# Dhia-naouali/dinov3-jax

Hardware: NVIDIA H100
Metric: global_crops_per_sec (higher is better)
Workload: dtype bf16

## Files before the change

### dinov3-jax_b200/csrc/attention.cu

```cuda
#include "ptx.cuh"
#include <climits>
#include <cstdlib>
#include "d3_internal.h"

namespace d3 {

constexpr float LOG2E = 1.4426950408889634f;
constexpr int SMEM_ALIGN = 1024;

__device__ __forceinline__ uint8_t* smem_base_1024(uint8_t* raw) {
  return reinterpret_cast<uint8_t*>((reinterpret_cast<uintptr_t>(raw) + 1023) & ~uintptr_t(1023));
}

struct AttnShape {
  int G;
  int span;
  int n_crops;
  int N;
  int nkb;
  int D;
  int H;
  float scale;
  const float* sin_t;
  const float* cos_t;
// ... 2 lines not shown

__device__ __forceinline__ uint32_t sw128_offset(int row, int col) {
  return (uint32_t)(row * 128 + ((((col >> 3) ^ (row & 7)) & 7) << 4) + (col & 7) * 2);
}

struct RowInfo { int g, klo, khi; bool ok; };
__device__ __forceinline__ RowInfo row_info(const AttnShape& sh, int c, int q) {
  RowInfo ri;
  ri.g = min(q / sh.N, sh.G - 1);
  ri.klo = ri.g * sh.N;
  ri.khi = ri.klo + sh.N;
  ri.ok = (q < sh.span) && (c * sh.G + ri.g < sh.n_crops);
  return ri;
}

template <int NI, int NO>
__device__ __forceinline__ void online_softmax(float (&s)[4 * NI], float (&o)[NO], float (&m)[2], float (&l)[2],
                                               const RowInfo (&ri)[2], int k0, int c2, float cs) {
  const int kb0 = k0 + c2;
  const bool full = k0 >= max(ri[0].klo, ri[1].klo) && k0 + 8 * NI <= min(ri[0].khi, ri[1].khi);
  float mx[2] = {-3.0e38f, -3.0e38f};
#pragma unroll
  for (int i = 0; i < NI; ++i)
#pragma unroll
    for (int j = 0; j < 4; ++j) {
      const int hh = j >> 1, kk = kb0 + 8 * i + (j & 1);
      if (full || (kk >= ri[hh].klo && kk < ri[hh].khi)) mx[hh] = fmaxf(mx[hh], s[4 * i + j]);
    }
  float corr[2], ms[2];
#pragma unroll
  for (int hh = 0; hh < 2; ++hh) {
    mx[hh] = fmaxf(mx[hh], __shfl_xor_sync(0xffffffffu, mx[hh], 1));
    mx[hh] = fmaxf(mx[hh], __shfl_xor_sync(0xffffffffu, mx[hh], 2));
    const float mn = fmaxf(m[hh], mx[hh]);
    corr[hh] = ex2_approx((m[hh] - mn) * cs);
    m[hh] = mn;
    ms[hh] = mn * cs;
    l[hh] *= corr[hh];
  }
#pragma unroll
  for (int i = 0; i < NI; ++i)
#pragma unroll
    for (int j = 0; j < 4; ++j) {
      const int hh = j >> 1, kk = kb0 + 8 * i + (j & 1);
      const float p = (full || (kk >= ri[hh].klo && kk < ri[hh].khi)) ? ex2_approx(fmaf(s[4 * i + j], cs, -ms[hh])) : 0.f;
      s[4 * i + j] = p;
      l[hh] += p;
      if (i < NO / 4) o[4 * i + j] *= corr[hh];
    }
}

template <int NO>
__device__ __forceinline__ void store_o_lse(const float (&o)[NO], float (&l)[2], const float (&m)[2], const RowInfo (&ri)[2],
                                            const AttnShape& sh, int c, int h, int row_base, int wq0, int r_in, int c2,
                                            __nv_bfloat16* O, float* LSE) {
#pragma unroll
  for (int hh = 0; hh < 2; ++hh) {
    l[hh] += __shfl_xor_sync(0xffffffffu, l[hh], 1);
    l[hh] += __shfl_xor_sync(0xffffffffu, l[hh], 2);
    const int q = wq0 + r_in + 8 * hh;
    if (!ri[hh].ok) continue;
    const float inv = 1.f / l[hh];
    __nv_bfloat16* dst = O + (size_t)(row_base + q) * sh.D + h * (2 * NO) + c2;
#pragma unroll
    for (int i = 0; i < NO / 4; ++i)
      *reinterpret_cast<uint32_t*>(dst + 8 * i) = pack_bf16(o[4 * i + 2 * hh] * inv, o[4 * i + 2 * hh + 1] * inv);
    if (LSE && c2 == 0)
      LSE[((size_t)(c * sh.G + ri[hh].g) * sh.H + h) * sh.N + (q - ri[hh].klo)] = m[hh] * sh.scale + logf(l[hh]);
  }
}

__host__ __device__ constexpr int fwd_smem(int nkb) { return SMEM_ALIGN + 16384 + 2 * nkb * 8192 + 8; }

__global__ void __launch_bounds__(256)
attn_fwd_kernel(const __grid_constant__ CUtensorMap tmQ, const __grid_constant__ CUtensorMap tmKV,
                __nv_bfloat16* __restrict__ O, float* __restrict__ LSE, const AttnShape sh) {
  extern __shared__ uint8_t smem_raw[];
  uint8_t* sQ = smem_base_1024(smem_raw);
  uint8_t* sK = sQ + 16384;
  uint8_t* sV = sK + sh.nkb * 8192;
  uint64_t* bar = reinterpret_cast<uint64_t*>(sV + sh.nkb * 8192);

  const int wg = threadIdx.x >> 7, t = threadIdx.x & 127;
  const int qt = blockIdx.x, h = blockIdx.y, c = blockIdx.z;
  const int q0 = qt * 128;
  const int row_base = c * sh.span;
  if (threadIdx.x == 0) {
    tma_prefetch_desc(&tmQ);
    tma_prefetch_desc(&tmKV);
    mbar_init(bar, 1);
    fence_mbar_init();
  }
  __syncthreads();
  if (threadIdx.x < 32 && elect_one()) {
    mbar_expect_tx(bar, 16384 + 2 * sh.nkb * 8192);
    tma_load_2d(&tmQ, bar, sQ, h * 64, row_base + q0);
    for (int b = 0; b < sh.nkb; ++b) {
      tma_load_2d(&tmKV, bar, sK + b * 8192, sh.D + h * 64, row_base + b * 64);
      tma_load_2d(&tmKV, bar, sV + b * 8192, 2 * sh.D + h * 64, row_base + b * 64);
    }
  }
  const int wq0 = q0 + wg * 64;
  if (wq0 >= sh.span) return;
  mbar_wait(bar, 0);

  const int r_in = 16 * (t >> 5) + ((t & 31) >> 2), c2 = 2 * (t & 3);
  RowInfo ri[2];
  ri[0] = row_info(sh, c, wq0 + r_in);
  ri[1] = row_info(sh, c, wq0 + r_in + 8);
  const int b_lo = (min(wq0 / sh.N, sh.G - 1) * sh.N) >> 6;
  const int b_hi = min(sh.nkb, ((min(min(wq0 + 63, sh.span - 1) / sh.N, sh.G - 1) + 1) * sh.N + 63) >> 6);
  const float cs = sh.scale * LOG2E;
  float m[2] = {-3.0e38f, -3.0e38f}, l[2] = {0.f, 0.f};
  float o[32];
#pragma unroll
  for (int i = 0; i < 32; ++i) o[i] = 0.f;
  const uint64_t qd = gmma_desc_sw128(smem_u32(sQ + wg * 8192), 16, 1024);

#pragma unroll 1
  for (int b = b_lo; b < b_hi; ++b) {
    float s[32];
    const uint64_t kd = gmma_desc_sw128(smem_u32(sK + b * 8192), 16, 1024);
    fence_regs(o);
    wgmma_fence();
#pragma unroll
    for (int k = 0; k < 4; ++k) wgmma_m64n64k16_ss<0, 0>(s, qd + 2 * k, kd + 2 * k, k > 0 ? 1u : 0u);
    wgmma_commit();
    wgmma_wait<0>();
    fence_regs(s);
    online_softmax<8>(s, o, m, l, ri, b * 64, c2, cs);
    uint32_t a[4][4];
#pragma unroll
    for (int kk = 0; kk < 4; ++kk)
#pragma unroll
      for (int e = 0; e < 4; ++e) a[kk][e] = pack_bf16(s[8 * kk + 2 * e], s[8 * kk + 2 * e + 1]);
    const uint64_t vd = gmma_desc_sw128(smem_u32(sV + b * 8192), 8192, 1024);
    fence_regs(o);
    wgmma_fence();
#pragma unroll
    for (int kk = 0; kk < 4; ++kk) wgmma_m64n64k16_rs<1>(o, a[kk], vd + 128 * kk, 1u);
    wgmma_commit();
    wgmma_wait<0>();
    fence_regs(o);
  }
  store_o_lse(o, l, m, ri, sh, c, h, row_base, wq0, r_in, c2, O, LSE);
}

template <int STAGES, int BYTES>
struct TileRing {
  static constexpr int SMEM = STAGES * BYTES + 2 * STAGES * 8;
  uint8_t* buf;
  uint64_t* full;
  uint64_t* empty;

  __device__ __forceinline__ explicit TileRing(uint8_t* base)
// ... 258 lines not shown
#pragma unroll
  for (int kk = 0; kk < 8; ++kk)
#pragma unroll
    for (int e = 0; e < 4; ++e) a[kk][e] = pack_bf16(dp[8 * kk + 2 * e], dp[8 * kk + 2 * e + 1]);
  const uint64_t kd = gmma_desc_sw128(smem_u32(sK), 8192, 1024);
  fence_regs(dq);
  wgmma_fence();
#pragma unroll
  for (int kk = 0; kk < 8; ++kk) wgmma_m64n64k16_rs<1>(dq, a[kk], kd + 128 * kk, 1u);
  wgmma_commit();
  wgmma_wait<0>();
  fence_regs(dq);
}


__host__ __device__ constexpr int bwd_fused_smem(int n_t) {
  return n_t * 32768 * 2 + 32768 + (n_t > 1 ? 2 * 32768 : 0) + n_t * 128 * 8 + 2 * n_t * 8;
}

__device__ __forceinline__ uint64_t desc_here(const void* p, uint32_t lbo, uint32_t sbo) {
  uint32_t a;
  asm volatile("mov.b32 %0, %1;" : "=r"(a) : "r"(smem_u32(p)));
  return gmma_desc_sw128(a, lbo, sbo);
}

template <int R>
__device__ __forceinline__ void fence_frag(uint32_t (&a)[R][4]) {
#pragma unroll
  for (int i = 0; i < R; ++i)
#pragma unroll
    for (int e = 0; e < 4; ++e) asm volatile("" : "+r"(a[i][e])::"memory");
}

__global__ void __launch_bounds__(256, 1)
attn_bwd_fused_kernel(const __grid_constant__ CUtensorMap tmQKV, const __grid_constant__ CUtensorMap tmDO,
                      const float* __restrict__ LSE, const float* __restrict__ Delta, __nv_bfloat16* __restrict__ dQKV,
                      const AttnShape sh) {
  extern __shared__ __align__(1024) uint8_t smem_al[];
  const int nT = (sh.span + 127) / 128;
  uint8_t* sKV = smem_al;
  uint8_t* sQDO = sKV + nT * 32768;
  uint8_t* sDS = sQDO + nT * 32768;
  uint8_t* sDS0 = sDS + 32768;
  float* sDQ = reinterpret_cast<float*>(sDS0 + 32768);
  float* sLSE = reinterpret_cast<float*>(sDS + (nT > 1 ? 3 * 32768 : 32768));
  float* sDel = sLSE + nT * 128;
  uint64_t* bar_kv = reinterpret_cast<uint64_t*>(sDel + nT * 128);
  uint64_t* bar_q = bar_kv + nT;

  const int wg = threadIdx.x >> 7, t = threadIdx.x & 127;
  const int r_in = 16 * (t >> 5) + ((t & 31) >> 2), c2 = 2 * (t & 3);
  const int h = blockIdx.x, c = blockIdx.y;
  const int row_base = c * sh.span;
  if (threadIdx.x == 0) {
    tma_prefetch_desc(&tmQKV);
    tma_prefetch_desc(&tmDO);
    for (int i = 0; i < 2 * nT; ++i) mbar_init(bar_kv + i, 1);
    fence_mbar_init();
  }
  __syncthreads();
  if (threadIdx.x < 32 && elect_one()) {
    for (int i = 0; i < nT; ++i) {
      mbar_expect_tx(bar_kv + i, 32768);
      tma_load_2d(&tmQKV, bar_kv + i, sKV + i * 32768, sh.D + h * 64, row_base + i * 128);
      tma_load_2d(&tmQKV, bar_kv + i, sKV + i * 32768 + 16384, 2 * sh.D + h * 64, row_base + i * 128);
      mbar_expect_tx(bar_q + i, 32768);
      tma_load_2d(&tmQKV, bar_q + i, sQDO + i * 32768, h * 64, row_base + i * 128);
      tma_load_2d(&tmDO, bar_q + i, sQDO + i * 32768 + 16384, h * 64, row_base + i * 128);
    }
  }
  for (int q = threadIdx.x; q < nT * 128; q += 256) {
    const RowInfo ri = row_info(sh, c, q);
    const size_t stat = ((size_t)(c * sh.G + ri.g) * sh.H + h) * sh.N + (q - ri.klo);
    sLSE[q] = ri.ok ? LSE[stat] * LOG2E : 0.f;
    sDel[q] = ri.ok ? Delta[stat] : 0.f;
  }
  __syncthreads();

  const float cs = sh.scale * LOG2E;
  int pair = 0;
#pragma unroll 1
  for (int kt = 0; kt < nT; ++kt) {
    mbar_wait(bar_kv + kt, 0);
    const uint8_t* sK = sKV + kt * 32768;
    const uint8_t* sV = sK + 16384;
    int lo[2], hi[2];
#pragma unroll
    for (int hh = 0; hh < 2; ++hh) {
      const RowInfo ri = row_info(sh, c, kt * 128 + wg * 64 + r_in + 8 * hh);
      lo[hh] = ri.ok ? ri.klo : 0;
      hi[hh] = ri.ok ? ri.khi : 0;
    }
    float dk[32], dv[32];
#pragma unroll 1
    for (int qt = 0; qt < nT; ++qt, ++pair) {
      mbar_wait(bar_q + qt, 0);
      const uint8_t* sQt = sQDO + qt * 32768;
      const uint8_t* sDOt = sQt + 16384;
      const bool defer = nT == 2 && kt == 0 && qt == 0;
      uint8_t* stash = defer ? sDS0 : sDS;
      uint32_t pa[2][4][4], da[2][4][4];
#pragma unroll
      for (int hf = 0; hf < 2; ++hf) {
        float s[32], dp[32];
        {
          const uint64_t kd = desc_here(sK + wg * 8192, 16, 1024);
          const uint64_t vd = desc_here(sV + wg * 8192, 16, 1024);
          const uint64_t qd = desc_here(sQt + hf * 8192, 16, 1024);
          const uint64_t dod = desc_here(sDOt + hf * 8192, 16, 1024);
          wgmma_fence();
#pragma unroll
          for (int k = 0; k < 4; ++k) {
            wgmma_m64n64k16_ss<0, 0>(s, kd + 2 * k, qd + 2 * k, k > 0 ? 1u : 0u);
            wgmma_m64n64k16_ss<0, 0>(dp, vd + 2 * k, dod + 2 * k, k > 0 ? 1u : 0u);
          }
          wgmma_commit();
          wgmma_wait<0>();
          fence_regs(s);
          fence_regs(dp);
          if (hf == 1) { fence_frag(pa[0]); fence_frag(da[0]); }
        }
        const float* lse2 = sLSE + qt * 128 + hf * 64;
        const float* del = sDel + qt * 128 + hf * 64;
#pragma unroll
        for (int i = 0; i < 8; ++i) {
          const int col = 8 * i + c2;
          const float2 l2 = *reinterpret_cast<const float2*>(lse2 + col);
          const float2 dl = *reinterpret_cast<const float2*>(del + col);
          const int q = qt * 128 + hf * 64 + col;
          float pv[4], dv4[4];
#pragma unroll
          for (int j = 0; j < 4; ++j) {
            const int hh = j >> 1, qq = q + (j & 1);
            const bool ok = qq >= lo[hh] && qq < hi[hh];
            const float p = ok ? ex2_approx(fmaf(s[4 * i + j], cs, -((j & 1) ? l2.y : l2.x))) : 0.f;
            dv4[j] = ok ? (p * sh.scale) * (dp[4 * i + j] - ((j & 1) ? dl.y : dl.x)) : 0.f;
            pv[j] = p;
          }
          pa[hf][i >> 1][2 * (i & 1)] = pack_bf16(pv[0], pv[1]);
          pa[hf][i >> 1][2 * (i & 1) + 1] = pack_bf16(pv[2], pv[3]);
          da[hf][i >> 1][2 * (i & 1)] = pack_bf16(dv4[0], dv4[1]);
          da[hf][i >> 1][2 * (i & 1) + 1] = pack_bf16(dv4[2], dv4[3]);
        }
        if (hf == 0 && pair > 1) named_bar_sync(1, 256);
#pragma unroll
        for (int hh = 0; hh < 2; ++hh)
#pragma unroll
          for (int i = 0; i < 8; ++i) {
            const uint32_t off = hf * 16384 + sw128_offset(wg * 64 + r_in + 8 * hh, 8 * i + c2);
            *reinterpret_cast<uint32_t*>(stash + off) = da[hf][i >> 1][2 * (i & 1) + hh];
          }
        {
          const uint64_t dod = desc_here(sDOt, 8192, 1024);
          const uint64_t qd = desc_here(sQt, 8192, 1024);
          const uint32_t acc_on = (qt > 0 || hf > 0) ? 1u : 0u;
          if (acc_on) { fence_regs(dk); fence_regs(dv); }
          wgmma_fence();
#pragma unroll
          for (int kk = 0; kk < 4; ++kk) {
            const int ks = 4 * hf + kk;
            wgmma_m64n64k16_rs<1>(dv, pa[hf][kk], dod + 128 * ks, (acc_on || kk > 0) ? 1u : 0u);
            wgmma_m64n64k16_rs<1>(dk, da[hf][kk], qd + 128 * ks, (acc_on || kk > 0) ? 1u : 0u);
          }
          wgmma_commit();
        }
      }
      fence_proxy_async_smem();
      if (defer) {
        wgmma_wait<0>();
        fence_regs(dk);
        fence_regs(dv);
        fence_frag(pa[1]);
        fence_frag(da[1]);
        continue;
      }
      named_bar_sync(2, 256);
      const bool from_partial = nT == 2 && kt == 1 && qt == 1;
      float dq[32];
      float4* part = reinterpret_cast<float4*>(sDQ) + wg * 8 * 128 + t;
      if (from_partial) {
#pragma unroll
        for (int j = 0; j < 8; ++j) {
          const float4 v = part[j * 128];
          dq[4 * j] = v.x; dq[4 * j + 1] = v.y; dq[4 * j + 2] = v.z; dq[4 * j + 3] = v.w;
        }
      }
      {
        const uint64_t sd = desc_here(sDS + wg * 16384, 16384, 1024);
        const uint64_t kbd = desc_here(sK, 8192, 1024);
        fence_regs(dq);
        wgmma_fence();
#pragma unroll
        for (int kk = 0; kk < 8; ++kk)
          wgmma_m64n64k16_ss<1, 1>(dq, sd + 128 * kk, kbd + 128 * kk, (from_partial || kk > 0) ? 1u : 0u);
        if (nT == 2 && kt == 1 && qt == 0) {
          const uint64_t sd0 = desc_here(sDS0 + wg * 16384, 16384, 1024);
          const uint64_t k0d = desc_here(sKV, 8192, 1024);
#pragma unroll
          for (int kk = 0; kk < 8; ++kk) wgmma_m64n64k16_ss<1, 1>(dq, sd0 + 128 * kk, k0d + 128 * kk, 1u);
        }
        wgmma_commit();
        wgmma_wait<0>();
        fence_regs(dq);
        fence_regs(dk);
        fence_regs(dv);
        fence_frag(pa[1]);
        fence_frag(da[1]);
      }
      if (nT == 2 && kt == 0) {
#pragma unroll
        for (int j = 0; j < 8; ++j) part[j * 128] = make_float4(dq[4 * j], dq[4 * j + 1], dq[4 * j + 2], dq[4 * j + 3]);
      } else {
        store_grad_rows(dq, sh, c, row_base, qt * 128 + wg * 64, r_in, c2, h, 0, true, dQKV);
      }
    }
    store_grad_rows(dk, sh, c, row_base, kt * 128 + wg * 64, r_in, c2, h, 1, true, dQKV);
    store_grad_rows(dv, sh, c, row_base, kt * 128 + wg * 64, r_in, c2, h, 2, false, dQKV);
  }
}

using DkdvRing = TileRing<DKDV_STAGES, 32768>;
constexpr int DKDV_SMEM = SMEM_ALIGN + 2 * 16384 + 2 * 32768 + DkdvRing::SMEM + 8;
using DqRing = TileRing<DQ_STAGES, 32768>;
constexpr int DQ_SMEM = SMEM_ALIGN + 2 * 16384 + DqRing::SMEM + 8;

__global__ void __launch_bounds__(RING_THREADS, 1)
attn_bwd_dkdv_kernel(const __grid_constant__ CUtensorMap tmQKV, const __grid_constant__ CUtensorMap tmDO,
                     const float* __restrict__ LSE, const float* __restrict__ Delta, __nv_bfloat16* __restrict__ dQKV,
                     const AttnShape sh) {
  extern __shared__ uint8_t smem_raw[];
  uint8_t* sK = smem_base_1024(smem_raw);
  uint8_t* sV = sK + 16384;
// ... 483 lines not shown
  if ((rc = make_map(&tdo, d_o, T, D, D, 128))) return rc;
  __nv_bfloat16* dq = (__nv_bfloat16*)dqkv;
  if (hd128) {
    if ((rc = launch<attn_bwd_dkdv_hd128_kernel>(grid, RING_THREADS, HD128_BWD_SMEM, HD128_BWD_SMEM, st, tqkv, tdo, lse,
                                                 delta_scratch, dq, s)))
      return rc;
    return launch<attn_bwd_dq_hd128_kernel>(grid, RING_THREADS, HD128_BWD_SMEM, HD128_BWD_SMEM, st, tqkv, tdo, lse,
                                            delta_scratch, dq, s);
  }
  if (streamed) {
    if ((rc = launch<attn_bwd_dkdv_kernel>(grid, RING_THREADS, DKDV_SMEM, DKDV_SMEM, st, tqkv, tdo, lse, delta_scratch, dq,
                                           s)))
      return rc;
    return launch<attn_bwd_dq_kernel>(grid, RING_THREADS, DQ_SMEM, DQ_SMEM, st, tqkv, tdo, lse, delta_scratch, dq, s);
  }
  return launch<attn_bwd_fused_kernel>(dim3(H, (n_crops + s.G - 1) / s.G), 256, bwd_fused_smem((s.span + 127) / 128),
                                       bwd_fused_smem(ATTN_BWD_RESIDENT_SPAN / 128), st, tqkv, tdo, lse, delta_scratch,
                                       dq, s);
}

}
```

### dinov3-jax_b200/csrc/ptx.cuh

```cuda
#pragma once
#include <cuda.h>
#include <cuda_runtime.h>
#include <cuda_bf16.h>
#include <stdint.h>

namespace d3 {

__device__ __forceinline__ uint32_t smem_u32(const void* p) {
  return static_cast<uint32_t>(__cvta_generic_to_shared(p));
}
__device__ __forceinline__ uint32_t lane_id() { return threadIdx.x & 31; }
__device__ __forceinline__ bool elect_one() {
  uint32_t pred;
  asm volatile("{\n\t.reg .pred p;\n\telect.sync _|p, 0xffffffff;\n\tselp.u32 %0, 1, 0, p;\n\t}" : "=r"(pred));
  return pred != 0;
}

__device__ __forceinline__ void mbar_init(uint64_t* bar, uint32_t count) {
  asm volatile("mbarrier.init.shared::cta.b64 [%0], %1;" ::"r"(smem_u32(bar)), "r"(count) : "memory");
}
__device__ __forceinline__ void fence_mbar_init() {
  asm volatile("fence.mbarrier_init.release.cluster;" ::: "memory");
}
__device__ __forceinline__ void mbar_expect_tx(uint64_t* bar, uint32_t bytes) {
// ... 107 lines not shown
__device__ __forceinline__ void wgmma_m64n32k16_ss(float (&d)[16], uint64_t da, uint64_t db, uint32_t scale_d) {
  asm volatile(
      "{\n\t.reg .pred p;\n\tsetp.ne.b32 p, %18, 0;\n\t"
      "wgmma.mma_async.sync.aligned.m64n32k16.f32.bf16.bf16 {%0, %1, %2, %3, %4, %5, %6, %7, %8, %9, %10, %11, %12, %13, %14, %15}, %16, %17, p, 1, 1, %19, %20;\n\t}"
      : "+f"(d[0]), "+f"(d[1]), "+f"(d[2]), "+f"(d[3]), "+f"(d[4]), "+f"(d[5]), "+f"(d[6]), "+f"(d[7]), "+f"(d[8]), "+f"(d[9]), "+f"(d[10]), "+f"(d[11]), "+f"(d[12]), "+f"(d[13]), "+f"(d[14]), "+f"(d[15])
      : "l"(da), "l"(db), "r"(scale_d), "n"(TA), "n"(TB));
}
template <int TA, int TB>
__device__ __forceinline__ void wgmma_m64n64k16_ss(float (&d)[32], uint64_t da, uint64_t db, uint32_t scale_d) {
  asm volatile(
      "{\n\t.reg .pred p;\n\tsetp.ne.b32 p, %34, 0;\n\t"
      "wgmma.mma_async.sync.aligned.m64n64k16.f32.bf16.bf16 {%0, %1, %2, %3, %4, %5, %6, %7, %8, %9, %10, %11, %12, %13, %14, %15, %16, %17, %18, %19, %20, %21, %22, %23, %24, %25, %26, %27, %28, %29, %30, %31}, %32, %33, p, 1, 1, %35, %36;\n\t}"
      : "+f"(d[0]), "+f"(d[1]), "+f"(d[2]), "+f"(d[3]), "+f"(d[4]), "+f"(d[5]), "+f"(d[6]), "+f"(d[7]), "+f"(d[8]), "+f"(d[9]), "+f"(d[10]), "+f"(d[11]), "+f"(d[12]), "+f"(d[13]), "+f"(d[14]), "+f"(d[15]), "+f"(d[16]), "+f"(d[17]), "+f"(d[18]), "+f"(d[19]), "+f"(d[20]), "+f"(d[21]), "+f"(d[22]), "+f"(d[23]), "+f"(d[24]), "+f"(d[25]), "+f"(d[26]), "+f"(d[27]), "+f"(d[28]), "+f"(d[29]), "+f"(d[30]), "+f"(d[31])
      : "l"(da), "l"(db), "r"(scale_d), "n"(TA), "n"(TB));
}
template <int TA, int TB>
__device__ __forceinline__ void wgmma_m64n128k16_ss(float (&d)[64], uint64_t da, uint64_t db, uint32_t scale_d) {
  asm volatile(
      "{\n\t.reg .pred p;\n\tsetp.ne.b32 p, %66, 0;\n\t"
      "wgmma.mma_async.sync.aligned.m64n128k16.f32.bf16.bf16 {%0, %1, %2, %3, %4, %5, %6, %7, %8, %9, %10, %11, %12, %13, %14, %15, %16, %17, %18, %19, %20, %21, %22, %23, %24, %25, %26, %27, %28, %29, %30, %31, %32, %33, %34, %35, %36, %37, %38, %39, %40, %41, %42, %43, %44, %45, %46, %47, %48, %49, %50, %51, %52, %53, %54, %55, %56, %57, %58, %59, %60, %61, %62, %63}, %64, %65, p, 1, 1, %67, %68;\n\t}"
      : "+f"(d[0]), "+f"(d[1]), "+f"(d[2]), "+f"(d[3]), "+f"(d[4]), "+f"(d[5]), "+f"(d[6]), "+f"(d[7]), "+f"(d[8]), "+f"(d[9]), "+f"(d[10]), "+f"(d[11]), "+f"(d[12]), "+f"(d[13]), "+f"(d[14]), "+f"(d[15]), "+f"(d[16]), "+f"(d[17]), "+f"(d[18]), "+f"(d[19]), "+f"(d[20]), "+f"(d[21]), "+f"(d[22]), "+f"(d[23]), "+f"(d[24]), "+f"(d[25]), "+f"(d[26]), "+f"(d[27]), "+f"(d[28]), "+f"(d[29]), "+f"(d[30]), "+f"(d[31]), "+f"(d[32]), "+f"(d[33]), "+f"(d[34]), "+f"(d[35]), "+f"(d[36]), "+f"(d[37]), "+f"(d[38]), "+f"(d[39]), "+f"(d[40]), "+f"(d[41]), "+f"(d[42]), "+f"(d[43]), "+f"(d[44]), "+f"(d[45]), "+f"(d[46]), "+f"(d[47]), "+f"(d[48]), "+f"(d[49]), "+f"(d[50]), "+f"(d[51]), "+f"(d[52]), "+f"(d[53]), "+f"(d[54]), "+f"(d[55]), "+f"(d[56]), "+f"(d[57]), "+f"(d[58]), "+f"(d[59]), "+f"(d[60]), "+f"(d[61]), "+f"(d[62]), "+f"(d[63])
      : "l"(da), "l"(db), "r"(scale_d), "n"(TA), "n"(TB));
}
template <int TA, int TB>
__device__ __forceinline__ void wgmma_m64n256k16_ss(float (&d)[128], uint64_t da, uint64_t db, uint32_t scale_d) {
  asm volatile(
      "{\n\t.reg .pred p;\n\tsetp.ne.b32 p, %130, 0;\n\t"
      "wgmma.mma_async.sync.aligned.m64n256k16.f32.bf16.bf16 {%0, %1, %2, %3, %4, %5, %6, %7, %8, %9, %10, %11, %12, %13, %14, %15, %16, %17, %18, %19, %20, %21, %22, %23, %24, %25, %26, %27, %28, %29, %30, %31, %32, %33, %34, %35, %36, %37, %38, %39, %40, %41, %42, %43, %44, %45, %46, %47, %48, %49, %50, %51, %52, %53, %54, %55, %56, %57, %58, %59, %60, %61, %62, %63, %64, %65, %66, %67, %68, %69, %70, %71, %72, %73, %74, %75, %76, %77, %78, %79, %80, %81, %82, %83, %84, %85, %86, %87, %88, %89, %90, %91, %92, %93, %94, %95, %96, %97, %98, %99, %100, %101, %102, %103, %104, %105, %106, %107, %108, %109, %110, %111, %112, %113, %114, %115, %116, %117, %118, %119, %120, %121, %122, %123, %124, %125, %126, %127}, %128, %129, p, 1, 1, %131, %132;\n\t}"
      : "+f"(d[0]), "+f"(d[1]), "+f"(d[2]), "+f"(d[3]), "+f"(d[4]), "+f"(d[5]), "+f"(d[6]), "+f"(d[7]), "+f"(d[8]), "+f"(d[9]), "+f"(d[10]), "+f"(d[11]), "+f"(d[12]), "+f"(d[13]), "+f"(d[14]), "+f"(d[15]), "+f"(d[16]), "+f"(d[17]), "+f"(d[18]), "+f"(d[19]), "+f"(d[20]), "+f"(d[21]), "+f"(d[22]), "+f"(d[23]), "+f"(d[24]), "+f"(d[25]), "+f"(d[26]), "+f"(d[27]), "+f"(d[28]), "+f"(d[29]), "+f"(d[30]), "+f"(d[31]), "+f"(d[32]), "+f"(d[33]), "+f"(d[34]), "+f"(d[35]), "+f"(d[36]), "+f"(d[37]), "+f"(d[38]), "+f"(d[39]), "+f"(d[40]), "+f"(d[41]), "+f"(d[42]), "+f"(d[43]), "+f"(d[44]), "+f"(d[45]), "+f"(d[46]), "+f"(d[47]), "+f"(d[48]), "+f"(d[49]), "+f"(d[50]), "+f"(d[51]), "+f"(d[52]), "+f"(d[53]), "+f"(d[54]), "+f"(d[55]), "+f"(d[56]), "+f"(d[57]), "+f"(d[58]), "+f"(d[59]), "+f"(d[60]), "+f"(d[61]), "+f"(d[62]), "+f"(d[63]), "+f"(d[64]), "+f"(d[65]), "+f"(d[66]), "+f"(d[67]), "+f"(d[68]), "+f"(d[69]), "+f"(d[70]), "+f"(d[71]), "+f"(d[72]), "+f"(d[73]), "+f"(d[74]), "+f"(d[75]), "+f"(d[76]), "+f"(d[77]), "+f"(d[78]), "+f"(d[79]), "+f"(d[80]), "+f"(d[81]), "+f"(d[82]), "+f"(d[83]), "+f"(d[84]), "+f"(d[85]), "+f"(d[86]), "+f"(d[87]), "+f"(d[88]), "+f"(d[89]), "+f"(d[90]), "+f"(d[91]), "+f"(d[92]), "+f"(d[93]), "+f"(d[94]), "+f"(d[95]), "+f"(d[96]), "+f"(d[97]), "+f"(d[98]), "+f"(d[99]), "+f"(d[100]), "+f"(d[101]), "+f"(d[102]), "+f"(d[103]), "+f"(d[104]), "+f"(d[105]), "+f"(d[106]), "+f"(d[107]), "+f"(d[108]), "+f"(d[109]), "+f"(d[110]), "+f"(d[111]), "+f"(d[112]), "+f"(d[113]), "+f"(d[114]), "+f"(d[115]), "+f"(d[116]), "+f"(d[117]), "+f"(d[118]), "+f"(d[119]), "+f"(d[120]), "+f"(d[121]), "+f"(d[122]), "+f"(d[123]), "+f"(d[124]), "+f"(d[125]), "+f"(d[126]), "+f"(d[127])
      : "l"(da), "l"(db), "r"(scale_d), "n"(TA), "n"(TB));
// ... 62 lines not shown
```

Baseline: 550.2.

## Pipeline attention forward KV loads per block and make backward persistent with double buffering

The forward kernel now gives each KV block its own mbarrier, so compute on early blocks can start while later blocks are still loading. It also trims the last partial block using narrower wgmma N shapes and fewer PV steps. The backward fused kernel is templated on tile count and becomes persistent for single-tile spans, double-buffering the next item's Q/K/V/dO and the LSE/Delta stats (now fetched with cp.async) behind the current item's compute. In exchange the forward loop drops the per-group block range and scans all KV blocks with masking, which adds work when several groups share a span. The backward path also uses more shared memory for the second buffer.

Result: no change. 551.5 (median of 6 runs) (+0.2%).

```diff
diff --git a/dinov3-jax_b200/csrc/attention.cu b/dinov3-jax_b200/csrc/attention.cu
--- a/dinov3-jax_b200/csrc/attention.cu
+++ b/dinov3-jax_b200/csrc/attention.cu
@@ -40,14 +40,15 @@
   return ri;
 }
 
-template <int NI, int NO>
+template <int NI, int NO, int NW = NI>
 __device__ __forceinline__ void online_softmax(float (&s)[4 * NI], float (&o)[NO], float (&m)[2], float (&l)[2],
                                                const RowInfo (&ri)[2], int k0, int c2, float cs) {
+  static_assert(NW >= 1 && NW <= NI, "1 .. NI column groups in range");
   const int kb0 = k0 + c2;
-  const bool full = k0 >= max(ri[0].klo, ri[1].klo) && k0 + 8 * NI <= min(ri[0].khi, ri[1].khi);
+  const bool full = k0 >= max(ri[0].klo, ri[1].klo) && k0 + 8 * NW <= min(ri[0].khi, ri[1].khi);
   float mx[2] = {-3.0e38f, -3.0e38f};
 #pragma unroll
-  for (int i = 0; i < NI; ++i)
+  for (int i = 0; i < NW; ++i)
 #pragma unroll
     for (int j = 0; j < 4; ++j) {
       const int hh = j >> 1, kk = kb0 + 8 * i + (j & 1);
@@ -69,9 +70,13 @@
 #pragma unroll
     for (int j = 0; j < 4; ++j) {
       const int hh = j >> 1, kk = kb0 + 8 * i + (j & 1);
-      const float p = (full || (kk >= ri[hh].klo && kk < ri[hh].khi)) ? ex2_approx(fmaf(s[4 * i + j], cs, -ms[hh])) : 0.f;
-      s[4 * i + j] = p;
-      l[hh] += p;
+      if (i < NW) {
+        const float p = (full || (kk >= ri[hh].klo && kk < ri[hh].khi)) ? ex2_approx(fmaf(s[4 * i + j], cs, -ms[hh])) : 0.f;
+        s[4 * i + j] = p;
+        l[hh] += p;
+      } else {
+        s[4 * i + j] = 0.f;
+      }
       if (i < NO / 4) o[4 * i + j] *= corr[hh];
     }
 }
@@ -96,7 +101,19 @@
   }
 }
 
-__host__ __device__ constexpr int fwd_smem(int nkb) { return SMEM_ALIGN + 16384 + 2 * nkb * 8192 + 8; }
+__host__ __device__ constexpr int fwd_smem(int nkb) { return SMEM_ALIGN + 16384 + 2 * nkb * 8192 + 8 * nkb; }
+
+template <int NW>
+__device__ __forceinline__ void fwd_s_block(float (&s)[32], uint64_t qd, uint64_t kd) {
+#pragma unroll
+  for (int k = 0; k < 4; ++k) wgmma_m64nNk16_ss<8 * NW, 0, 0>(s, qd + 2 * k, kd + 2 * k, k > 0 ? 1u : 0u);
+}
+
+template <int NK>
+__device__ __forceinline__ void fwd_pv_block(float (&o)[32], const uint32_t (&a)[4][4], uint64_t vd) {
+#pragma unroll
+  for (int kk = 0; kk < NK; ++kk) wgmma_m64n64k16_rs<1>(o, a[kk], vd + 128 * kk, 1u);
+}
 
 __global__ void __launch_bounds__(256)
 attn_fwd_kernel(const __grid_constant__ CUtensorMap tmQ, const __grid_constant__ CUtensorMap tmKV,
@@ -114,28 +131,26 @@
   if (threadIdx.x == 0) {
     tma_prefetch_desc(&tmQ);
     tma_prefetch_desc(&tmKV);
-    mbar_init(bar, 1);
+    for (int b = 0; b < sh.nkb; ++b) mbar_init(bar + b, 1);
     fence_mbar_init();
   }
   __syncthreads();
   if (threadIdx.x < 32 && elect_one()) {
-    mbar_expect_tx(bar, 16384 + 2 * sh.nkb * 8192);
-    tma_load_2d(&tmQ, bar, sQ, h * 64, row_base + q0);
     for (int b = 0; b < sh.nkb; ++b) {
-      tma_load_2d(&tmKV, bar, sK + b * 8192, sh.D + h * 64, row_base + b * 64);
-      tma_load_2d(&tmKV, bar, sV + b * 8192, 2 * sh.D + h * 64, row_base + b * 64);
+      mbar_expect_tx(bar + b, (b == 0 ? 16384 : 0) + 2 * 8192);
+      if (b == 0) tma_load_2d(&tmQ, bar, sQ, h * 64, row_base + q0);
+      tma_load_2d(&tmKV, bar + b, sK + b * 8192, sh.D + h * 64, row_base + b * 64);
+      tma_load_2d(&tmKV, bar + b, sV + b * 8192, 2 * sh.D + h * 64, row_base + b * 64);
     }
   }
   const int wq0 = q0 + wg * 64;
   if (wq0 >= sh.span) return;
-  mbar_wait(bar, 0);
 
   const int r_in = 16 * (t >> 5) + ((t & 31) >> 2), c2 = 2 * (t & 3);
   RowInfo ri[2];
   ri[0] = row_info(sh, c, wq0 + r_in);
   ri[1] = row_info(sh, c, wq0 + r_in + 8);
-  const int b_lo = (min(wq0 / sh.N, sh.G - 1) * sh.N) >> 6;
-  const int b_hi = min(sh.nkb, ((min(min(wq0 + 63, sh.span - 1) / sh.N, sh.G - 1) + 1) * sh.N + 63) >> 6);
+  const int nw_last = (sh.span - (sh.nkb - 1) * 64 + 7) >> 3;
   const float cs = sh.scale * LOG2E;
   float m[2] = {-3.0e38f, -3.0e38f}, l[2] = {0.f, 0.f};
   float o[32];
@@ -144,27 +159,51 @@
   const uint64_t qd = gmma_desc_sw128(smem_u32(sQ + wg * 8192), 16, 1024);
 
 #pragma unroll 1
-  for (int b = b_lo; b < b_hi; ++b) {
+  for (int b = 0; b < sh.nkb; ++b) {
+    mbar_wait(bar + b, 0);
+    const int nw = b + 1 < sh.nkb ? 8 : nw_last;
     float s[32];
     const uint64_t kd = gmma_desc_sw128(smem_u32(sK + b * 8192), 16, 1024);
     fence_regs(o);
     wgmma_fence();
-#pragma unroll
-    for (int k = 0; k < 4; ++k) wgmma_m64n64k16_ss<0, 0>(s, qd + 2 * k, kd + 2 * k, k > 0 ? 1u : 0u);
+    switch (nw) {
+      case 1: fwd_s_block<1>(s, qd, kd); break;
+      case 2: fwd_s_block<2>(s, qd, kd); break;
+      case 3: fwd_s_block<3>(s, qd, kd); break;
+      case 4: fwd_s_block<4>(s, qd, kd); break;
+      case 5: fwd_s_block<5>(s, qd, kd); break;
+      case 6: fwd_s_block<6>(s, qd, kd); break;
+      case 7: fwd_s_block<7>(s, qd, kd); break;
+      default: fwd_s_block<8>(s, qd, kd); break;
+    }
     wgmma_commit();
     wgmma_wait<0>();
     fence_regs(s);
-    online_softmax<8>(s, o, m, l, ri, b * 64, c2, cs);
+    switch (nw) {
+      case 1: online_softmax<8, 32, 1>(s, o, m, l, ri, b * 64, c2, cs); break;
+      case 2: online_softmax<8, 32, 2>(s, o, m, l, ri, b * 64, c2, cs); break;
+      case 3: online_softmax<8, 32, 3>(s, o, m, l, ri, b * 64, c2, cs); break;
+      case 4: online_softmax<8, 32, 4>(s, o, m, l, ri, b * 64, c2, cs); break;
+      case 5: online_softmax<8, 32, 5>(s, o, m, l, ri, b * 64, c2, cs); break;
+      case 6: online_softmax<8, 32, 6>(s, o, m, l, ri, b * 64, c2, cs); break;
+      case 7: online_softmax<8, 32, 7>(s, o, m, l, ri, b * 64, c2, cs); break;
+      default: online_softmax<8, 32, 8>(s, o, m, l, ri, b * 64, c2, cs); break;
+    }
     uint32_t a[4][4];
 #pragma unroll
     for (int kk = 0; kk < 4; ++kk)
 #pragma unroll
       for (int e = 0; e < 4; ++e) a[kk][e] = pack_bf16(s[8 * kk + 2 * e], s[8 * kk + 2 * e + 1]);
     const uint64_t vd = gmma_desc_sw128(smem_u32(sV + b * 8192), 8192, 1024);
+    const int n_pv = (nw + 1) >> 1;
     fence_regs(o);
     wgmma_fence();
-#pragma unroll
-    for (int kk = 0; kk < 4; ++kk) wgmma_m64n64k16_rs<1>(o, a[kk], vd + 128 * kk, 1u);
+    switch (n_pv) {
+      case 1: fwd_pv_block<1>(o, a, vd); break;
+      case 2: fwd_pv_block<2>(o, a, vd); break;
+      case 3: fwd_pv_block<3>(o, a, vd); break;
+      default: fwd_pv_block<4>(o, a, vd); break;
+    }
     wgmma_commit();
     wgmma_wait<0>();
     fence_regs(o);
@@ -453,8 +492,9 @@
 }
 
 
+__host__ __device__ constexpr int bwd_fused_bufs(int n_t) { return n_t == 1 ? 2 : 1; }
 __host__ __device__ constexpr int bwd_fused_smem(int n_t) {
-  return n_t * 32768 * 2 + 32768 + (n_t > 1 ? 2 * 32768 : 0) + n_t * 128 * 8 + 2 * n_t * 8;
+  return bwd_fused_bufs(n_t) * (n_t * 65536 + n_t * 128 * 8 + 2 * n_t * 8) + 32768 + (n_t > 1 ? 2 * 32768 : 0);
 }
 
 __device__ __forceinline__ uint64_t desc_here(const void* p, uint32_t lbo, uint32_t sbo) {
@@ -471,190 +511,212 @@
     for (int e = 0; e < 4; ++e) asm volatile("" : "+r"(a[i][e])::"memory");
 }
 
+template <int NT>
 __global__ void __launch_bounds__(256, 1)
 attn_bwd_fused_kernel(const __grid_constant__ CUtensorMap tmQKV, const __grid_constant__ CUtensorMap tmDO,
                       const float* __restrict__ LSE, const float* __restrict__ Delta, __nv_bfloat16* __restrict__ dQKV,
                       const AttnShape sh) {
   extern __shared__ __align__(1024) uint8_t smem_al[];
-  const int nT = (sh.span + 127) / 128;
-  uint8_t* sKV = smem_al;
-  uint8_t* sQDO = sKV + nT * 32768;
-  uint8_t* sDS = sQDO + nT * 32768;
+  constexpr int nT = NT, nB = bwd_fused_bufs(NT);
+  uint8_t* sDS = smem_al + nB * nT * 65536;
   uint8_t* sDS0 = sDS + 32768;
   float* sDQ = reinterpret_cast<float*>(sDS0 + 32768);
-  float* sLSE = reinterpret_cast<float*>(sDS + (nT > 1 ? 3 * 32768 : 32768));
-  float* sDel = sLSE + nT * 128;
-  uint64_t* bar_kv = reinterpret_cast<uint64_t*>(sDel + nT * 128);
-  uint64_t* bar_q = bar_kv + nT;
+  float* sStat = reinterpret_cast<float*>(sDS + (nT > 1 ? 3 * 32768 : 32768));
+  uint64_t* bar_kv = reinterpret_cast<uint64_t*>(sStat + nB * nT * 256);
+  uint64_t* bar_q = bar_kv + nB * nT;
 
   const int wg = threadIdx.x >> 7, t = threadIdx.x & 127;
   const int r_in = 16 * (t >> 5) + ((t & 31) >> 2), c2 = 2 * (t & 3);
-  const int h = blockIdx.x, c = blockIdx.y;
-  const int row_base = c * sh.span;
+  const int n_items = sh.H * ((sh.n_crops + sh.G - 1) / sh.G);
   if (threadIdx.x == 0) {
     tma_prefetch_desc(&tmQKV);
     tma_prefetch_desc(&tmDO);
-    for (int i = 0; i < 2 * nT; ++i) mbar_init(bar_kv + i, 1);
+    for (int i = 0; i < 2 * nB * nT; ++i) mbar_init(bar_kv + i, 1);
     fence_mbar_init();
   }
   __syncthreads();
-  if (threadIdx.x < 32 && elect_one()) {
-    for (int i = 0; i < nT; ++i) {
-      mbar_expect_tx(bar_kv + i, 32768);
-      tma_load_2d(&tmQKV, bar_kv + i, sKV + i * 32768, sh.D + h * 64, row_base + i * 128);
-      tma_load_2d(&tmQKV, bar_kv + i, sKV + i * 32768 + 16384, 2 * sh.D + h * 64, row_base + i * 128);
-      mbar_expect_tx(bar_q + i, 32768);
-      tma_load_2d(&tmQKV, bar_q + i, sQDO + i * 32768, h * 64, row_base + i * 128);
-      tma_load_2d(&tmDO, bar_q + i, sQDO + i * 32768 + 16384, h * 64, row_base + i * 128);
-    }
-  }
-  for (int q = threadIdx.x; q < nT * 128; q += 256) {
-    const RowInfo ri = row_info(sh, c, q);
-    const size_t stat = ((size_t)(c * sh.G + ri.g) * sh.H + h) * sh.N + (q - ri.klo);
-    sLSE[q] = ri.ok ? LSE[stat] * LOG2E : 0.f;
-    sDel[q] = ri.ok ? Delta[stat] : 0.f;
-  }
-  __syncthreads();
+  auto load_item = [&](int item, int u) {
+    const int h = item % sh.H, c = item / sh.H, row_base = c * sh.span;
+    if (threadIdx.x < 32 && elect_one()) {
+      uint8_t* sKV = smem_al + u * nT * 65536;
+      uint8_t* sQDO = sKV + nT * 32768;
+      for (int i = 0; i < nT; ++i) {
+        uint64_t* bkv = bar_kv + u * nT + i;
+        uint64_t* bq = bar_q + u * nT + i;
+        mbar_expect_tx(bkv, 32768);
+        tma_load_2d(&tmQKV, bkv, sKV + i * 32768, sh.D + h * 64, row_base + i * 128);
+        tma_load_2d(&tmQKV, bkv, sKV + i * 32768 + 16384, 2 * sh.D + h * 64, row_base + i * 128);
+        mbar_expect_tx(bq, 32768);
+        tma_load_2d(&tmQKV, bq, sQDO + i * 32768, h * 64, row_base + i * 128);
+        tma_load_2d(&tmDO, bq, sQDO + i * 32768 + 16384, h * 64, row_base + i * 128);
+      }
+    }
+    float* sLSE = sStat + u * nT * 256;
+    for (int q = threadIdx.x; q < nT * 128; q += 256) {
+      const RowInfo ri = row_info(sh, c, q);
+      const size_t stat = ri.ok ? ((size_t)(c * sh.G + ri.g) * sh.H + h) * sh.N + (q - ri.klo) : 0;
+      cp_async_4(sLSE + q, LSE + stat);
+      cp_async_4(sLSE + nT * 128 + q, Delta + stat);
+    }
+  };
+  if (blockIdx.x < n_items) load_item(blockIdx.x, 0);
 
   const float cs = sh.scale * LOG2E;
-  int pair = 0;
 #pragma unroll 1
-  for (int kt = 0; kt < nT; ++kt) {
-    mbar_wait(bar_kv + kt, 0);
-    const uint8_t* sK = sKV + kt * 32768;
-    const uint8_t* sV = sK + 16384;
-    int lo[2], hi[2];
-#pragma unroll
-    for (int hh = 0; hh < 2; ++hh) {
-      const RowInfo ri = row_info(sh, c, kt * 128 + wg * 64 + r_in + 8 * hh);
-      lo[hh] = ri.ok ? ri.klo : 0;
-      hi[hh] = ri.ok ? ri.khi : 0;
-    }
-    float dk[32], dv[32];
+  for (int item = blockIdx.x, it = 0; item < n_items && (NT == 1 || it == 0); item += gridDim.x, ++it) {
+    const int u = it % nB;
+    const uint32_t ph = (it / nB) & 1;
+    cp_async_wait_all();
+    __syncthreads();
+    if (nB > 1 && item + (int)gridDim.x < n_items) load_item(item + gridDim.x, u ^ 1);
+    const int h = item % sh.H, c = item / sh.H;
+    const int row_base = c * sh.span;
+    const uint8_t* sKV = smem_al + u * nT * 65536;
+    const uint8_t* sQDO = sKV + nT * 32768;
+    const float* sLSE = sStat + u * nT * 256;
+    const float* sDel = sLSE + nT * 128;
+    uint64_t* bkv = bar_kv + u * nT;
+    uint64_t* bq = bar_q + u * nT;
+    int pair = 0;
 #pragma unroll 1
-    for (int qt = 0; qt < nT; ++qt, ++pair) {
-      mbar_wait(bar_q + qt, 0);
-      const uint8_t* sQt = sQDO + qt * 32768;
-      const uint8_t* sDOt = sQt + 16384;
-      const bool defer = nT == 2 && kt == 0 && qt == 0;
-      uint8_t* stash = defer ? sDS0 : sDS;
-      uint32_t pa[2][4][4], da[2][4][4];
-#pragma unroll
-      for (int hf = 0; hf < 2; ++hf) {
-        float s[32], dp[32];
+    for (int kt = 0; kt < nT; ++kt) {
+      mbar_wait(bkv + kt, ph);
+      const uint8_t* sK = sKV + kt * 32768;
+      const uint8_t* sV = sK + 16384;
+      int lo[2], hi[2];
+#pragma unroll
+      for (int hh = 0; hh < 2; ++hh) {
+        const RowInfo ri = row_info(sh, c, kt * 128 + wg * 64 + r_in + 8 * hh);
+        lo[hh] = ri.ok ? ri.klo : 0;
+        hi[hh] = ri.ok ? ri.khi : 0;
+      }
+      float dk[32], dv[32];
+#pragma unroll 1
+      for (int qt = 0; qt < nT; ++qt, ++pair) {
+        mbar_wait(bq + qt, ph);
+        const uint8_t* sQt = sQDO + qt * 32768;
+        const uint8_t* sDOt = sQt + 16384;
+        const bool defer = nT == 2 && kt == 0 && qt == 0;
+        uint8_t* stash = defer ? sDS0 : sDS;
+        uint32_t pa[2][4][4], da[2][4][4];
+#pragma unroll
+        for (int hf = 0; hf < 2; ++hf) {
+          float s[32], dp[32];
+          {
+            const uint64_t kd = desc_here(sK + wg * 8192, 16, 1024);
+            const uint64_t vd = desc_here(sV + wg * 8192, 16, 1024);
+            const uint64_t qd = desc_here(sQt + hf * 8192, 16, 1024);
+            const uint64_t dod = desc_here(sDOt + hf * 8192, 16, 1024);
+            wgmma_fence();
+#pragma unroll
+            for (int k = 0; k < 4; ++k) {
+              wgmma_m64n64k16_ss<0, 0>(s, kd + 2 * k, qd + 2 * k, k > 0 ? 1u : 0u);
+              wgmma_m64n64k16_ss<0, 0>(dp, vd + 2 * k, dod + 2 * k, k > 0 ? 1u : 0u);
+            }
+            wgmma_commit();
+            wgmma_wait<0>();
+            fence_regs(s);
+            fence_regs(dp);
+            if (hf == 1) { fence_frag(pa[0]); fence_frag(da[0]); }
+          }
+          const float* lse2 = sLSE + qt * 128 + hf * 64;
+          const float* del = sDel + qt * 128 + hf * 64;
+#pragma unroll
+          for (int i = 0; i < 8; ++i) {
+            const int col = 8 * i + c2;
+            const float2 l2 = *reinterpret_cast<const float2*>(lse2 + col);
+            const float2 dl = *reinterpret_cast<const float2*>(del + col);
+            const int q = qt * 128 + hf * 64 + col;
+            float pv[4], dv4[4];
+#pragma unroll
+            for (int j = 0; j < 4; ++j) {
+              const int hh = j >> 1, qq = q + (j & 1);
+              const bool ok = qq >= lo[hh] && qq < hi[hh];
+              const float p = ok ? ex2_approx(fmaf(s[4 * i + j], cs, -(((j & 1) ? l2.y : l2.x) * LOG2E))) : 0.f;
+              dv4[j] = ok ? (p * sh.scale) * (dp[4 * i + j] - ((j & 1) ? dl.y : dl.x)) : 0.f;
+              pv[j] = p;
+            }
+            pa[hf][i >> 1][2 * (i & 1)] = pack_bf16(pv[0], pv[1]);
+            pa[hf][i >> 1][2 * (i & 1) + 1] = pack_bf16(pv[2], pv[3]);
+            da[hf][i >> 1][2 * (i & 1)] = pack_bf16(dv4[0], dv4[1]);
+            da[hf][i >> 1][2 * (i & 1) + 1] = pack_bf16(dv4[2], dv4[3]);
+          }
+          if (hf == 0 && pair > 1) named_bar_sync(1, 256);
+#pragma unroll
+          for (int hh = 0; hh < 2; ++hh)
+#pragma unroll
+            for (int i = 0; i < 8; ++i) {
+              const uint32_t off = hf * 16384 + sw128_offset(wg * 64 + r_in + 8 * hh, 8 * i + c2);
+              *reinterpret_cast<uint32_t*>(stash + off) = da[hf][i >> 1][2 * (i & 1) + hh];
+            }
+          {
+            const uint64_t dod = desc_here(sDOt, 8192, 1024);
+            const uint64_t qd = desc_here(sQt, 8192, 1024);
+            const uint32_t acc_on = (qt > 0 || hf > 0) ? 1u : 0u;
+            if (acc_on) { fence_regs(dk); fence_regs(dv); }
+            wgmma_fence();
+#pragma unroll
+            for (int kk = 0; kk < 4; ++kk) {
+              const int ks = 4 * hf + kk;
+              wgmma_m64n64k16_rs<1>(dv, pa[hf][kk], dod + 128 * ks, (acc_on || kk > 0) ? 1u : 0u);
+              wgmma_m64n64k16_rs<1>(dk, da[hf][kk], qd + 128 * ks, (acc_on || kk > 0) ? 1u : 0u);
+            }
+            wgmma_commit();
+          }
+        }
+        fence_proxy_async_smem();
+        if (defer) {
+          wgmma_wait<0>();
+          fence_regs(dk);
+          fence_regs(dv);
+          fence_frag(pa[1]);
+          fence_frag(da[1]);
+          continue;
+        }
+        named_bar_sync(2, 256);
+        const bool from_partial = nT == 2 && kt == 1 && qt == 1;
+        float dq[32];
+        float4* part = reinterpret_cast<float4*>(sDQ) + wg * 8 * 128 + t;
+        if (from_partial) {
+#pragma unroll
+          for (int j = 0; j < 8; ++j) {
+            const float4 v = part[j * 128];
+            dq[4 * j] = v.x; dq[4 * j + 1] = v.y; dq[4 * j + 2] = v.z; dq[4 * j + 3] = v.w;
+          }
+        }
         {
-          const uint64_t kd = desc_here(sK + wg * 8192, 16, 1024);
-          const uint64_t vd = desc_here(sV + wg * 8192, 16, 1024);
-          const uint64_t qd = desc_here(sQt + hf * 8192, 16, 1024);
-          const uint64_t dod = desc_here(sDOt + hf * 8192, 16, 1024);
+          const uint64_t sd = desc_here(sDS + wg * 16384, 16384, 1024);
+          const uint64_t kbd = desc_here(sK, 8192, 1024);
+          fence_regs(dq);
           wgmma_fence();
 #pragma unroll
-          for (int k = 0; k < 4; ++k) {
-            wgmma_m64n64k16_ss<0, 0>(s, kd + 2 * k, qd + 2 * k, k > 0 ? 1u : 0u);
-            wgmma_m64n64k16_ss<0, 0>(dp, vd + 2 * k, dod + 2 * k, k > 0 ? 1u : 0u);
+          for (int kk = 0; kk < 8; ++kk)
+            wgmma_m64n64k16_ss<1, 1>(dq, sd + 128 * kk, kbd + 128 * kk, (from_partial || kk > 0) ? 1u : 0u);
+          if (nT == 2 && kt == 1 && qt == 0) {
+            const uint64_t sd0 = desc_here(sDS0 + wg * 16384, 16384, 1024);
+            const uint64_t k0d = desc_here(sKV, 8192, 1024);
+#pragma unroll
+            for (int kk = 0; kk < 8; ++kk) wgmma_m64n64k16_ss<1, 1>(dq, sd0 + 128 * kk, k0d + 128 * kk, 1u);
           }
           wgmma_commit();
           wgmma_wait<0>();
-          fence_regs(s);
-          fence_regs(dp);
-          if (hf == 1) { fence_frag(pa[0]); fence_frag(da[0]); }
+          fence_regs(dq);
+          fence_regs(dk);
+          fence_regs(dv);
+          fence_frag(pa[1]);
+          fence_frag(da[1]);
         }
-        const float* lse2 = sLSE + qt * 128 + hf * 64;
-        const float* del = sDel + qt * 128 + hf * 64;
-#pragma unroll
-        for (int i = 0; i < 8; ++i) {
-          const int col = 8 * i + c2;
-          const float2 l2 = *reinterpret_cast<const float2*>(lse2 + col);
-          const float2 dl = *reinterpret_cast<const float2*>(del + col);
-          const int q = qt * 128 + hf * 64 + col;
-          float pv[4], dv4[4];
-#pragma unroll
-          for (int j = 0; j < 4; ++j) {
-            const int hh = j >> 1, qq = q + (j & 1);
-            const bool ok = qq >= lo[hh] && qq < hi[hh];
-            const float p = ok ? ex2_approx(fmaf(s[4 * i + j], cs, -((j & 1) ? l2.y : l2.x))) : 0.f;
-            dv4[j] = ok ? (p * sh.scale) * (dp[4 * i + j] - ((j & 1) ? dl.y : dl.x)) : 0.f;
-            pv[j] = p;
-          }
-          pa[hf][i >> 1][2 * (i & 1)] = pack_bf16(pv[0], pv[1]);
-          pa[hf][i >> 1][2 * (i & 1) + 1] = pack_bf16(pv[2], pv[3]);
-          da[hf][i >> 1][2 * (i & 1)] = pack_bf16(dv4[0], dv4[1]);
-          da[hf][i >> 1][2 * (i & 1) + 1] = pack_bf16(dv4[2], dv4[3]);
-        }
-        if (hf == 0 && pair > 1) named_bar_sync(1, 256);
-#pragma unroll
-        for (int hh = 0; hh < 2; ++hh)
-#pragma unroll
-          for (int i = 0; i < 8; ++i) {
-            const uint32_t off = hf * 16384 + sw128_offset(wg * 64 + r_in + 8 * hh, 8 * i + c2);
-            *reinterpret_cast<uint32_t*>(stash + off) = da[hf][i >> 1][2 * (i & 1) + hh];
-          }
-        {
-          const uint64_t dod = desc_here(sDOt, 8192, 1024);
-          const uint64_t qd = desc_here(sQt, 8192, 1024);
-          const uint32_t acc_on = (qt > 0 || hf > 0) ? 1u : 0u;
-          if (acc_on) { fence_regs(dk); fence_regs(dv); }
-          wgmma_fence();
-#pragma unroll
-          for (int kk = 0; kk < 4; ++kk) {
-            const int ks = 4 * hf + kk;
-            wgmma_m64n64k16_rs<1>(dv, pa[hf][kk], dod + 128 * ks, (acc_on || kk > 0) ? 1u : 0u);
-            wgmma_m64n64k16_rs<1>(dk, da[hf][kk], qd + 128 * ks, (acc_on || kk > 0) ? 1u : 0u);
-          }
-          wgmma_commit();
+        if (nT == 2 && kt == 0) {
+#pragma unroll
+          for (int j = 0; j < 8; ++j)
+            part[j * 128] = make_float4(dq[4 * j], dq[4 * j + 1], dq[4 * j + 2], dq[4 * j + 3]);
+        } else {
+          store_grad_rows(dq, sh, c, row_base, qt * 128 + wg * 64, r_in, c2, h, 0, true, dQKV);
         }
       }
-      fence_proxy_async_smem();
-      if (defer) {
-        wgmma_wait<0>();
-        fence_regs(dk);
-        fence_regs(dv);
-        fence_frag(pa[1]);
-        fence_frag(da[1]);
-        continue;
-      }
-      named_bar_sync(2, 256);
-      const bool from_partial = nT == 2 && kt == 1 && qt == 1;
-      float dq[32];
-      float4* part = reinterpret_cast<float4*>(sDQ) + wg * 8 * 128 + t;
-      if (from_partial) {
-#pragma unroll
-        for (int j = 0; j < 8; ++j) {
-          const float4 v = part[j * 128];
-          dq[4 * j] = v.x; dq[4 * j + 1] = v.y; dq[4 * j + 2] = v.z; dq[4 * j + 3] = v.w;
-        }
-      }
-      {
-        const uint64_t sd = desc_here(sDS + wg * 16384, 16384, 1024);
-        const uint64_t kbd = desc_here(sK, 8192, 1024);
-        fence_regs(dq);
-        wgmma_fence();
-#pragma unroll
-        for (int kk = 0; kk < 8; ++kk)
-          wgmma_m64n64k16_ss<1, 1>(dq, sd + 128 * kk, kbd + 128 * kk, (from_partial || kk > 0) ? 1u : 0u);
-        if (nT == 2 && kt == 1 && qt == 0) {
-          const uint64_t sd0 = desc_here(sDS0 + wg * 16384, 16384, 1024);
-          const uint64_t k0d = desc_here(sKV, 8192, 1024);
-#pragma unroll
-          for (int kk = 0; kk < 8; ++kk) wgmma_m64n64k16_ss<1, 1>(dq, sd0 + 128 * kk, k0d + 128 * kk, 1u);
-        }
-        wgmma_commit();
-        wgmma_wait<0>();
-        fence_regs(dq);
-        fence_regs(dk);
-        fence_regs(dv);
-        fence_frag(pa[1]);
-        fence_frag(da[1]);
-      }
-      if (nT == 2 && kt == 0) {
-#pragma unroll
-        for (int j = 0; j < 8; ++j) part[j * 128] = make_float4(dq[4 * j], dq[4 * j + 1], dq[4 * j + 2], dq[4 * j + 3]);
-      } else {
-        store_grad_rows(dq, sh, c, row_base, qt * 128 + wg * 64, r_in, c2, h, 0, true, dQKV);
-      }
-    }
-    store_grad_rows(dk, sh, c, row_base, kt * 128 + wg * 64, r_in, c2, h, 1, true, dQKV);
-    store_grad_rows(dv, sh, c, row_base, kt * 128 + wg * 64, r_in, c2, h, 2, false, dQKV);
+      store_grad_rows(dk, sh, c, row_base, kt * 128 + wg * 64, r_in, c2, h, 1, true, dQKV);
+      store_grad_rows(dv, sh, c, row_base, kt * 128 + wg * 64, r_in, c2, h, 2, false, dQKV);
+    }
   }
 }
 
@@ -1168,9 +1230,20 @@
       return rc;
     return launch<attn_bwd_dq_kernel>(grid, RING_THREADS, DQ_SMEM, DQ_SMEM, st, tqkv, tdo, lse, delta_scratch, dq, s);
   }
-  return launch<attn_bwd_fused_kernel>(dim3(H, (n_crops + s.G - 1) / s.G), 256, bwd_fused_smem((s.span + 127) / 128),
-                                       bwd_fused_smem(ATTN_BWD_RESIDENT_SPAN / 128), st, tqkv, tdo, lse, delta_scratch,
-                                       dq, s);
-}
-
-}
+  const int nT = (s.span + 127) / 128;
+  long items = (long)H * ((n_crops + s.G - 1) / s.G);
+  if (items > INT_MAX) return set_error(D3_ERR_ARG, "d3_attn_bwd: H * crop groups must be below 2^31");
+  if (nT == 1) {
+    int dev = 0, sms = 0;
+    if (cudaGetDevice(&dev) != cudaSuccess || cudaDeviceGetAttribute(&sms, cudaDevAttrMultiProcessorCount, dev) != cudaSuccess)
+      return set_error(D3_ERR_CUDA, "d3_attn_bwd: SM count");
+    items = items < sms ? items : sms;
+  }
+  if (nT == 1)
+    return launch<attn_bwd_fused_kernel<1>>(dim3((unsigned)items), 256, bwd_fused_smem(1), bwd_fused_smem(1), st, tqkv,
+                                            tdo, lse, delta_scratch, dq, s);
+  return launch<attn_bwd_fused_kernel<2>>(dim3((unsigned)items), 256, bwd_fused_smem(2), bwd_fused_smem(2), st, tqkv, tdo,
+                                          lse, delta_scratch, dq, s);
+}
+
+}
diff --git a/dinov3-jax_b200/csrc/ptx.cuh b/dinov3-jax_b200/csrc/ptx.cuh
--- a/dinov3-jax_b200/csrc/ptx.cuh
+++ b/dinov3-jax_b200/csrc/ptx.cuh
@@ -145,6 +145,54 @@
       : "+f"(d[0]), "+f"(d[1]), "+f"(d[2]), "+f"(d[3]), "+f"(d[4]), "+f"(d[5]), "+f"(d[6]), "+f"(d[7]), "+f"(d[8]), "+f"(d[9]), "+f"(d[10]), "+f"(d[11]), "+f"(d[12]), "+f"(d[13]), "+f"(d[14]), "+f"(d[15]), "+f"(d[16]), "+f"(d[17]), "+f"(d[18]), "+f"(d[19]), "+f"(d[20]), "+f"(d[21]), "+f"(d[22]), "+f"(d[23]), "+f"(d[24]), "+f"(d[25]), "+f"(d[26]), "+f"(d[27]), "+f"(d[28]), "+f"(d[29]), "+f"(d[30]), "+f"(d[31])
       : "l"(da), "l"(db), "r"(scale_d), "n"(TA), "n"(TB));
 }
+template <int N, int TA, int TB>
+__device__ __forceinline__ void wgmma_m64nNk16_ss(float (&d)[32], uint64_t da, uint64_t db, uint32_t scale_d) {
+  static_assert(N % 8 == 0 && N >= 8 && N <= 64, "N = 8 .. 64, a multiple of 8");
+  if constexpr (N == 8)
+    asm volatile(
+        "{\n\t.reg .pred p;\n\tsetp.ne.b32 p, %6, 0;\n\t"
+        "wgmma.mma_async.sync.aligned.m64n8k16.f32.bf16.bf16 {%0, %1, %2, %3}, %4, %5, p, 1, 1, %7, %8;\n\t}"
+        : "+f"(d[0]), "+f"(d[1]), "+f"(d[2]), "+f"(d[3])
+        : "l"(da), "l"(db), "r"(scale_d), "n"(TA), "n"(TB));
+  else if constexpr (N == 16)
+    asm volatile(
+        "{\n\t.reg .pred p;\n\tsetp.ne.b32 p, %10, 0;\n\t"
+        "wgmma.mma_async.sync.aligned.m64n16k16.f32.bf16.bf16 {%0, %1, %2, %3, %4, %5, %6, %7}, %8, %9, p, 1, 1, %11, %12;\n\t}"
+        : "+f"(d[0]), "+f"(d[1]), "+f"(d[2]), "+f"(d[3]), "+f"(d[4]), "+f"(d[5]), "+f"(d[6]), "+f"(d[7])
+        : "l"(da), "l"(db), "r"(scale_d), "n"(TA), "n"(TB));
+  else if constexpr (N == 24)
+    asm volatile(
+        "{\n\t.reg .pred p;\n\tsetp.ne.b32 p, %14, 0;\n\t"
+        "wgmma.mma_async.sync.aligned.m64n24k16.f32.bf16.bf16 {%0, %1, %2, %3, %4, %5, %6, %7, %8, %9, %10, %11}, %12, %13, p, 1, 1, %15, %16;\n\t}"
+        : "+f"(d[0]), "+f"(d[1]), "+f"(d[2]), "+f"(d[3]), "+f"(d[4]), "+f"(d[5]), "+f"(d[6]), "+f"(d[7]), "+f"(d[8]), "+f"(d[9]), "+f"(d[10]), "+f"(d[11])
+        : "l"(da), "l"(db), "r"(scale_d), "n"(TA), "n"(TB));
+  else if constexpr (N == 32)
+    asm volatile(
+        "{\n\t.reg .pred p;\n\tsetp.ne.b32 p, %18, 0;\n\t"
+        "wgmma.mma_async.sync.aligned.m64n32k16.f32.bf16.bf16 {%0, %1, %2, %3, %4, %5, %6, %7, %8, %9, %10, %11, %12, %13, %14, %15}, %16, %17, p, 1, 1, %19, %20;\n\t}"
+        : "+f"(d[0]), "+f"(d[1]), "+f"(d[2]), "+f"(d[3]), "+f"(d[4]), "+f"(d[5]), "+f"(d[6]), "+f"(d[7]), "+f"(d[8]), "+f"(d[9]), "+f"(d[10]), "+f"(d[11]), "+f"(d[12]), "+f"(d[13]), "+f"(d[14]), "+f"(d[15])
+        : "l"(da), "l"(db), "r"(scale_d), "n"(TA), "n"(TB));
+  else if constexpr (N == 40)
+    asm volatile(
+        "{\n\t.reg .pred p;\n\tsetp.ne.b32 p, %22, 0;\n\t"
+        "wgmma.mma_async.sync.aligned.m64n40k16.f32.bf16.bf16 {%0, %1, %2, %3, %4, %5, %6, %7, %8, %9, %10, %11, %12, %13, %14, %15, %16, %17, %18, %19}, %20, %21, p, 1, 1, %23, %24;\n\t}"
+        : "+f"(d[0]), "+f"(d[1]), "+f"(d[2]), "+f"(d[3]), "+f"(d[4]), "+f"(d[5]), "+f"(d[6]), "+f"(d[7]), "+f"(d[8]), "+f"(d[9]), "+f"(d[10]), "+f"(d[11]), "+f"(d[12]), "+f"(d[13]), "+f"(d[14]), "+f"(d[15]), "+f"(d[16]), "+f"(d[17]), "+f"(d[18]), "+f"(d[19])
+        : "l"(da), "l"(db), "r"(scale_d), "n"(TA), "n"(TB));
+  else if constexpr (N == 48)
+    asm volatile(
+        "{\n\t.reg .pred p;\n\tsetp.ne.b32 p, %26, 0;\n\t"
+        "wgmma.mma_async.sync.aligned.m64n48k16.f32.bf16.bf16 {%0, %1, %2, %3, %4, %5, %6, %7, %8, %9, %10, %11, %12, %13, %14, %15, %16, %17, %18, %19, %20, %21, %22, %23}, %24, %25, p, 1, 1, %27, %28;\n\t}"
+        : "+f"(d[0]), "+f"(d[1]), "+f"(d[2]), "+f"(d[3]), "+f"(d[4]), "+f"(d[5]), "+f"(d[6]), "+f"(d[7]), "+f"(d[8]), "+f"(d[9]), "+f"(d[10]), "+f"(d[11]), "+f"(d[12]), "+f"(d[13]), "+f"(d[14]), "+f"(d[15]), "+f"(d[16]), "+f"(d[17]), "+f"(d[18]), "+f"(d[19]), "+f"(d[20]), "+f"(d[21]), "+f"(d[22]), "+f"(d[23])
+        : "l"(da), "l"(db), "r"(scale_d), "n"(TA), "n"(TB));
+  else if constexpr (N == 56)
+    asm volatile(
+        "{\n\t.reg .pred p;\n\tsetp.ne.b32 p, %30, 0;\n\t"
+        "wgmma.mma_async.sync.aligned.m64n56k16.f32.bf16.bf16 {%0, %1, %2, %3, %4, %5, %6, %7, %8, %9, %10, %11, %12, %13, %14, %15, %16, %17, %18, %19, %20, %21, %22, %23, %24, %25, %26, %27}, %28, %29, p, 1, 1, %31, %32;\n\t}"
+        : "+f"(d[0]), "+f"(d[1]), "+f"(d[2]), "+f"(d[3]), "+f"(d[4]), "+f"(d[5]), "+f"(d[6]), "+f"(d[7]), "+f"(d[8]), "+f"(d[9]), "+f"(d[10]), "+f"(d[11]), "+f"(d[12]), "+f"(d[13]), "+f"(d[14]), "+f"(d[15]), "+f"(d[16]), "+f"(d[17]), "+f"(d[18]), "+f"(d[19]), "+f"(d[20]), "+f"(d[21]), "+f"(d[22]), "+f"(d[23]), "+f"(d[24]), "+f"(d[25]), "+f"(d[26]), "+f"(d[27])
+        : "l"(da), "l"(db), "r"(scale_d), "n"(TA), "n"(TB));
+  else
+    wgmma_m64n64k16_ss<TA, TB>(d, da, db, scale_d);
+}
 template <int TA, int TB>
 __device__ __forceinline__ void wgmma_m64n128k16_ss(float (&d)[64], uint64_t da, uint64_t db, uint32_t scale_d) {
   asm volatile(
```
